# rrwick/Badread

Hardware: AMD Instinct MI355X
Metric: simulated bases/sec (higher is better)
Workload: dtype u32

## Files before the change

### badread_amd/csrc/brx_kernels.h

```cpp
#ifndef BRX_KERNELS_H
#define BRX_KERNELS_H

#include <hip/hip_runtime.h>
#include <stdint.h>

#include "../../include/brx.h"
#include "../../include/brx_spec.h"
#include "brx_align.h"

#define BRX_ALIGN_INTERVAL 25
#define BRX_ALIGN_SIZE 1000
#ifndef BRX_MAX_BASE_SEGS
#define BRX_MAX_BASE_SEGS 64
#endif
#define BRX_OVF_SEGS 4096
#define BRX_OVF_LISTS 64

enum { SEG_REF = 0, SEG_ADAPTER = 1, SEG_RANDOM = 2, SEG_JUNK = 3 };
enum { PC_JUNK = 0, PC_RANDOM = 1, PC_REAL = 2, PC_HAIRPIN = 3 };

struct PSeg { uint32_t w0, start, len, dst; };
struct PPiece { uint32_t w0, left_over; uint64_t start, end; };

struct RS {
// ... 651 lines not shown
                uint8_t kmer[16];
#pragma unroll
                for (int j = 0; j < 16; ++j) kmer[j] = j < k ? F[ipos + j] : 0;
                live = dev_choose_alt(em, kmer, w[2], w[3], rep);
            }
            unsigned long long surv = __ballot(live);
            while (surv) {
                int l = __ffsll((long long)surv) - 1;
                surv &= surv - 1;
                const uint64_t i0 = wave_bcast_u64(ipos, l);
                const double scale = est * brx_sqrt(est);
                for (int j = 0; j < k; ++j) {
                    uint32_t mine = 0;
#pragma unroll
                    for (int jj = 0; jj < 16; ++jj) mine = (jj == j) ? rep[jj] : mine;
                    uint32_t w = wave_bcast_u32(mine, l);
                    if (!w) continue;
                    uint64_t pos = i0 + (uint64_t)j;
                    const uint32_t cur = uni(rp[pos]);
                    if (cur) continue;
                    if (lane == 0) rp[pos] = w;
                    __builtin_amdgcn_fence(__ATOMIC_RELEASE, "workgroup");
                    change += 1;
                    uint32_t len = (w >> 24) & 0x7Fu;
                    errors += (double)(len < 2 ? 1u : len - 1u) * scale;
                    if (change % BRX_ALIGN_INTERVAL == 0) {
                        uint32_t a = 0, b = n;
                        if (n > BRX_ALIGN_SIZE) {
                            uint32_t ww[4];
                            brx_draw4(d.seed, read, BRX_ST_WIN, (uint64_t)nalign, ww);
                            a = (uint32_t)brx_mulhi64(((uint64_t)ww[1] << 32) | ww[0], (uint64_t)n - BRX_ALIGN_SIZE + 1);
                            b = a + BRX_ALIGN_SIZE;
                        }
                        nalign += 1;
                        __builtin_amdgcn_s_waitcnt(0);
                        uint32_t cost = 0;
                        uint32_t tl = wave_join(em, F, rp, a, b, nullptr, &cost);
                        uint32_t ql = b - a;
                        uint64_t qpad = ((uint64_t)ql + 16 + 15) & ~15ull, tpad = ((uint64_t)tl + 16 + 15) & ~15ull;
                        int ncols = 0, nmatch = 0; bool nospace = false;
                        if (qpad + tpad + 64 > win_bytes) nospace = true;
                        else {
                            uint8_t *qb = win, *tbuf = win + qpad;
                            for (uint32_t x = lane; x < ql + 16; x += 64) qb[x] = x < ql ? F[a + x] : 0xFF;
                            for (uint32_t x = lane; x < 16; x += 64) tbuf[tl + x] = 0xFE;
                            wave_join(em, F, rp, a, b, tbuf, nullptr);
                            __builtin_amdgcn_fence(__ATOMIC_RELEASE, "workgroup");
                            __builtin_amdgcn_s_waitcnt(0);
                            uint2 *tb = reinterpret_cast<uint2 *>(win + qpad + tpad);
                            uint64_t cap = (win_bytes - qpad - tpad) / 8;
                            bool ok = brx_wave_align<1>(qb, (int)ql, tbuf, (int)tl, (int)cost, tb, cap, nullptr, &ncols, &nmatch, &nospace,
                                                     nullptr, aclk);
                            if (!ok && !nospace) s.status |= BRX_RS_BAND;
                        }
                        if (nospace) { if (lane == 0) atomicOr(&flags[0], 1u); }
                        double id = ncols ? (double)nmatch / (double)ncols : 0.0;
                        if (n <= BRX_ALIGN_SIZE) errors = (1.0 - id) * dn;
                        else {
                            double est_err = (1.0 - id) * dn;
                            double weight = (double)BRX_ALIGN_SIZE / dn;
                            errors = est_err * weight + errors * (1.0 - weight);
                        }
                    }
                }
                double est2 = 1.0 - errors / dn;
                if ((double)change > 0.9 * dn || est2 <= target) { loops += (uint64_t)l + 2; done = true; break; }
                est = est2;
            }
            if (done) break;
            loops += B;
            if (B < 64) { loops += 1; break; }
        }
        __builtin_amdgcn_s_waitcnt(0);
        uint32_t cost = 0;
        uint32_t m = wave_join(em, F, rp, 0, n, nullptr, &cost);
        uint32_t st = 0, et = 0;
        if (lane < k) { st = rep_len(rp[lane]); et = rep_len(rp[n - k + lane]); }
        st = wave_sum(st); et = wave_sum(et);
        if (lane == 0) {
            RS *o = &rs[r];
            o->status = s.status; o->m = m; o->ub = cost; o->start_trim = st; o->end_trim = et;
            o->loops = (uint32_t)loops; o->changes = change; o->naligns = nalign;
            o->units = 0;
            uint64_t *ck = clk + (uint64_t)r * 8;
            ck[0] = __builtin_amdgcn_s_memtime() - t_begin; ck[1] = aclk[0]; ck[2] = aclk[1];
        }
    }
}

#include "brx_mutate.h"
#include "brx_passes.h"
#include "brx_model.h"
#include "brx_gzip_dev.h"

__global__ void __launch_bounds__(64) k_scan_mut(uint32_t n, RS *rs, const uint32_t *list, uint64_t *totals) {
    const int lane = lane_id();
    uint64_t seq_run = 0, ops_run = 0;
    for (uint32_t base = 0; base < n; base += 64) {
        const uint32_t i = base + lane;
        const uint32_t r = i < n ? list[i] : 0u;
        uint32_t sb = 0, ob = 0;
        if (i < n && rs[r].n) {
            sb = 2u * ((rs[r].m + 16u + 15u) >> 4);
            ob = (rs[r].m + rs[r].n + 16u + 15u) >> 4;
        }
        uint32_t is = wave_incl_scan(sb), io = wave_incl_scan(ob);
        if (i < n) { rs[r].seq_off = (seq_run + is - sb) << 4; rs[r].ops_off = (ops_run + io - ob) << 4; }
        seq_run += wave_bcast_u32(is, 63); ops_run += wave_bcast_u32(io, 63);
    }
    if (lane == 0) { totals[0] = seq_run << 4; totals[1] = ops_run << 4; }
}

__device__ inline int64_t qs_lookup(const brx_qscore_model &qm, uint64_t key) {
    uint64_t h = key * 0x9E3779B97F4A7C15ull;
    uint32_t slot = (uint32_t)(h >> 32) & (qm.hash_size - 1);
    for (;;) {
        uint64_t kk = qm.d_hash_key[slot];
        if (kk == key) return (int64_t)qm.d_hash_row[slot];
        if (kk == ~0ull) return -1;
        slot = (slot + 1) & (qm.hash_size - 1);
    }
}

#define BRX_KL_RETRY 0x10000u
#define BRX_KL_FULL 0x20000u
#define BRX_KL_LANES 0x40000u
#define BRX_KL_QUAD 0x80000u
#include "brx_finlanes.h"
#include "brx_quad.h"

__global__ void __launch_bounds__(64) k_fin_join(BrxDev d, RS *rs, const uint32_t *order, uint32_t q_begin, uint32_t q_end, uint32_t *queue,
                                                  uint64_t seq_base, uint64_t ops_base, const uint8_t *Fbuf, const uint32_t *repl,
                                                  const PPiece *pieces, uint8_t *arena, const uint32_t *F2buf, int fin_lanes, int fin_quad) {
    const int lane = lane_id();
    const brx_error_model &em = d.em;
    for (;;) {
        const uint32_t qi = q_begin + wave_pop(queue);
        if (qi >= q_end) break;
        const uint32_t r = order[qi];
        const RS s = rs[r];
        if (s.n == 0) {
            if (lane == 0) { rs[r].seq_off = seq_base; rs[r].ops_off = ops_base; }
            continue;
        }
        uint8_t *seq = arena + seq_base + s.seq_off;
        wave_join(em, Fbuf + s.F_off, repl + s.F_off, 0, s.n, seq, nullptr);
        for (uint32_t x = lane; x < 16; x += 64) seq[s.m + x] = 0xFE;
        if (lane == 0) {
            const BrxGeom g = brx_make_geom((int)s.m, (int)s.n, (int)s.ub);
            bool junk = false, too_wide;
            if (!d.raw_mode) for (uint32_t i = 0; i < s.n_pieces; ++i) junk |= (pieces[s.piece_off + i].w0 & 3u) == PC_JUNK;
            RS *o = &rs[r];
            o->seq_off = seq_base + s.seq_off; o->ops_off = ops_base + s.ops_off;
            const bool acgt = F2buf[(s.F_off >> 4) + ((s.n + 15u) >> 4)] == 0u;
            const bool lanes = fin_lanes && !junk && acgt && brx_finl_blocks(s.m, s.n, s.ub) > 0;
            const bool quad = fin_quad && !lanes && acgt && g.G == 1 && (brx_quad_words(s.m, s.n, s.ub) & fin_quad) != 0;
            o->klass = (g.G ? (uint32_t)g.G : 0xFFFFu) | (junk ? BRX_KL_FULL : 0u) | (lanes ? BRX_KL_LANES : 0u) | (quad ? BRX_KL_QUAD : 0u);
            o->units = brx_final_units(s.m, s.n, s.ub, junk ? 0 : d.tb_hmul, &too_wide);
            if (too_wide) o->status = s.status | BRX_RS_BAND;
        }
    }
}

__global__ void __launch_bounds__(64, 4) k_fin_lanes(BrxDev d, RS *rs, const uint32_t *list, uint32_t n_list, unsigned long long *ctr,
                                                      const uint64_t *slabs, uint32_t *retries, const uint8_t *Fbuf, uint8_t *seqbuf, uint8_t *opsbuf,
                                                      uint8_t *slab_base, uint64_t *clk) {
    const int lane = lane_id();
    const uint32_t n_groups = (n_list + 63u) >> 6;
    const uint64_t first = uni((uint64_t)atomicAdd(ctr, lane == 0 ? ((1ull << 32) | 1ull) : 0ull));
    uint32_t gi = (uint32_t)first;
    if (gi >= n_groups) return;
    const uint32_t ticket = (uint32_t)(first >> 32);
    const uint64_t slab_at = slabs[ticket], tb_cap = slabs[ticket + 1] - slab_at;
    uint2 *tb = reinterpret_cast<uint2 *>(slab_base) + slab_at;
    for (; gi < n_groups; gi = (uint32_t)uni((uint64_t)atomicAdd(ctr, lane == 0 ? 1ull : 0ull))) {
        const uint32_t idx = gi * 64u + (uint32_t)lane;
        bool valid = idx < n_list;
        const uint32_t r = valid ? list[idx] : 0u;
        RS s;
        if (valid) s = rs[r];
        const uint64_t t_begin = __builtin_amdgcn_s_memtime();
        const uint32_t n = valid ? s.n : 0u, m = valid ? s.m : 0u;
        const uint32_t blocks = wave_max_u32(valid ? (uint32_t)brx_finl_blocks(m, n, s.ub) : 0u);
        const bool fits = brx_finl_units(wave_max_u32(n), blocks) <= tb_cap;
        const uint8_t *F = Fbuf + (valid ? s.F_off : 0ull);
        const uint8_t *seq = seqbuf + (valid ? s.seq_off : 0ull);
        uint8_t *ops_end = opsbuf + (valid ? s.ops_off + (uint64_t)n + (uint64_t)m : 0ull);
        uint32_t ncols = 0, nmatch = 0; bool ok = false;
        brx_lanes_final(valid && fits, seq, (int)m, F, (int)n, valid ? (int)s.ub : 0, tb, ops_end, &ncols, &nmatch, &ok);
        if (valid) {
            RS *o = &rs[r];
            if (!ok) {
                o->klass = (s.klass & ~BRX_KL_LANES) | BRX_KL_RETRY;
                atomicAdd(retries, 1u);
                clk[(uint64_t)r * 8 + 2] = 1;
            } else {
                o->status = s.status;
                o->n_cols = ncols; o->n_match = nmatch;
            }
            uint64_t *ck = clk + (uint64_t)r * 8;
            ck[3] = __builtin_amdgcn_s_memtime() - t_begin; ck[7] = (uint64_t)(s.klass & 0xFFFFu) | 0x20000u;
        }
        __builtin_amdgcn_fence(__ATOMIC_RELEASE, "workgroup");
        __builtin_amdgcn_s_waitcnt(0);
    }
}

template <int G>
__global__ void __launch_bounds__(64, 4) k_fin_quad(BrxDev d, RS *rs, const uint32_t *list, uint32_t n_list, unsigned long long *ctr,
                                                     const uint64_t *slabs, uint32_t *retries, const uint8_t *Fbuf, uint8_t *seqbuf,
                                                     uint8_t *opsbuf, uint8_t *slab_base, uint64_t *clk) {
    const int lane = lane_id();
    const int row = lane >> 4;
    const uint32_t n_groups = (n_list + 3u) >> 2;
    const uint64_t first = uni((uint64_t)atomicAdd(ctr, lane == 0 ? ((1ull << 32) | 1ull) : 0ull));
    uint32_t gi = (uint32_t)first;
    if (gi >= n_groups) return;
    const uint32_t ticket = (uint32_t)(first >> 32);
    const uint64_t slab_at = slabs[ticket], tb_cap = slabs[ticket + 1] - slab_at;
    uint2 *tb = reinterpret_cast<uint2 *>(slab_base) + slab_at;
    for (; gi < n_groups; gi = (uint32_t)uni((uint64_t)atomicAdd(ctr, lane == 0 ? 1ull : 0ull))) {
        const uint32_t idx = gi * 4u + (uint32_t)row;
        const bool valid = idx < n_list;
        const uint32_t r = valid ? list[idx] : 0u;
        RS s;
        if (valid) s = rs[r];
        const uint64_t t_begin = __builtin_amdgcn_s_memtime();
        const uint32_t n = valid ? s.n : 0u, m = valid ? s.m : 0u;
        const uint8_t *F = Fbuf + (valid ? s.F_off : 0ull);
        const uint8_t *seq = seqbuf + (valid ? s.seq_off : 0ull);
        uint8_t *ops_end = opsbuf + (valid ? s.ops_off + (uint64_t)n + (uint64_t)m : 0ull);
        int ncols = 0, nmatch = 0, st = 1;
        brx_quad_align<G>(valid && m > 0 && n > 0, seq, (int)m, F, (int)n, valid ? (int)s.ub : 0,
                          (valid && !(s.klass & BRX_KL_FULL)) ? d.tb_hmul : 0, tb, tb_cap, ops_end, &ncols, &nmatch, &st);
        if (valid && (lane & 15) == 0) {
            RS *o = &rs[r];
            if (st != 0) {
                o->klass = (s.klass & ~BRX_KL_QUAD) | BRX_KL_RETRY;
                atomicAdd(retries, 1u);
                clk[(uint64_t)r * 8 + 2] = 1;
            } else {
                o->status = s.status;
                o->n_cols = (uint32_t)ncols; o->n_match = (uint32_t)nmatch;
            }
            uint64_t *ck = clk + (uint64_t)r * 8;
            ck[3] = __builtin_amdgcn_s_memtime() - t_begin; ck[7] = (uint64_t)(s.klass & 0xFFFFu) | 0x10000u;
        }
        __builtin_amdgcn_fence(__ATOMIC_RELEASE, "workgroup");
        __builtin_amdgcn_s_waitcnt(0);
    }
}

#ifndef BRX_FIN4_WAVES
#define BRX_FIN4_WAVES 4
#endif
template <int MAXG, int GLO, int GHI>
#ifndef BRX_FIN1_WAVES
#define BRX_FIN1_WAVES 5
#endif
#ifndef BRX_FIN2_WAVES
#define BRX_FIN2_WAVES 4
#endif
__global__ void __launch_bounds__(64, (MAXG == 1 ? BRX_FIN1_WAVES : MAXG == 2 ? BRX_FIN2_WAVES : MAXG == 4 ? BRX_FIN4_WAVES : 1)) k_fin_align(BrxDev d, RS *rs, const uint32_t *list, uint32_t n_list,
                                                   unsigned long long *ctr, const uint64_t *slabs, uint32_t *retries, int phase, const uint8_t *Fbuf,
                                                   uint8_t *seqbuf, uint8_t *opsbuf, uint8_t *slab_base, uint64_t *clk) {
    const int lane = lane_id();
    const uint64_t first = uni((uint64_t)atomicAdd(ctr, lane == 0 ? ((1ull << 32) | 1ull) : 0ull));
    uint32_t qi = (uint32_t)first;
    if (qi >= n_list) return;
    const uint32_t ticket = (uint32_t)(first >> 32);
    const uint64_t slab_at = slabs[ticket], tb_cap = slabs[ticket + 1] - slab_at;
    uint2 *tb = reinterpret_cast<uint2 *>(slab_base) + slab_at;
    for (; qi < n_list; qi = (uint32_t)uni((uint64_t)atomicAdd(ctr, lane == 0 ? 1ull : 0ull))) {
        const uint32_t r = list[qi];
        const RS s = rs[r];
        const int klass = (int)(s.klass & 0xFFFFu);
        const uint64_t t_begin = __builtin_amdgcn_s_memtime();
        uint64_t aclk[2] = {0, 0};
        const uint32_t n = s.n, m = s.m;
        const uint8_t *F = Fbuf + s.F_off;
        uint8_t *seq = seqbuf + s.seq_off;
        uint8_t *ops_end = opsbuf + s.ops_off + (uint64_t)n + (uint64_t)m;
        int ncols = 0, nmatch = 0; bool nospace = false;
        const bool ok = brx_wave_align<MAXG, (GLO < MAXG ? GLO : MAXG)>(seq, (int)m, F, (int)n, (int)s.ub, tb, tb_cap, ops_end, &ncols, &nmatch,
                                             &nospace, nullptr, aclk, (phase == 0 && !(s.klass & BRX_KL_FULL)) ? d.tb_hmul : 0);
        if (lane == 0) {
            RS *o = &rs[r];
            if (!ok && phase == 0) {
                o->klass = s.klass | BRX_KL_RETRY;
                atomicAdd(retries, 1u);
                clk[(uint64_t)r * 8 + 2] = 1;
            } else {
                o->status = s.status | (ok ? 0u : BRX_RS_BAND);
                o->n_cols = (uint32_t)ncols; o->n_match = (uint32_t)nmatch;
            }
            uint64_t *ck = clk + (uint64_t)r * 8;
            ck[3] = __builtin_amdgcn_s_memtime() - t_begin; ck[4] = aclk[0]; ck[5] = aclk[1];
            ck[7] = (uint64_t)klass;
        }
    }
}

#define BRX_QS_HOT_MAX 128
#define BRX_QS_PEND 128
__global__ void __launch_bounds__(64) k_fin_qscore(BrxDev d, RS *rs, const uint32_t *order, uint32_t q_begin, uint32_t q_end,
                                                    uint32_t *queue, int phase, int klo, int khi, uint8_t *seqbuf, const uint8_t *opsbuf,
                                                    uint64_t *clk) {
    __shared__ uint32_t qhist[256];
    __shared__ uint32_t hot_thr[BRX_QS_HOT_MAX], hot_score[BRX_QS_HOT_MAX];
    __shared__ uint8_t hot_idx[256];
    __shared__ uint32_t pend_sp[BRX_QS_PEND], pend_h[BRX_QS_PEND], pend_c[BRX_QS_PEND];
    __shared__ uint32_t draw_lds[512];
    const int lane = lane_id();
    const brx_qscore_model &qm = d.qm;
    uint32_t hot_n = 0;
    {
        const int64_t row = qs_lookup(qm, (uint64_t)qm.k << 56);
        if (row >= 0) {
            const uint32_t e0 = qm.d_row_off[row], e1 = qm.d_row_off[row + 1];
            if (e1 - e0 <= BRX_QS_HOT_MAX) {
                hot_n = e1 - e0;
                for (uint32_t x = lane; x < hot_n; x += 64) { hot_thr[x] = qm.d_thr[e0 + x]; hot_score[x] = qm.d_score[e0 + x]; }
            }
        }
        __syncthreads();
        for (uint32_t b = lane; b < 256u && hot_n; b += 64) {
            const uint32_t u = b << 24;
            uint32_t e = 0, hi_ = hot_n - 1;
            while (e < hi_) { const uint32_t mid = (e + hi_) >> 1; if (u < hot_thr[mid]) hi_ = mid; else e = mid + 1; }
            hot_idx[b] = (uint8_t)e;
        }
        __syncthreads();
    }
    for (;;) {
        const uint32_t qi = q_begin + wave_pop(queue);
        if (qi >= q_end) break;
        const uint32_t r = order[qi];
        RS s = rs[r];
        if (s.n == 0) continue;
        if (((s.klass & BRX_KL_RETRY) != 0u) != (phase != 0)) continue;
        if ((int)(s.klass & 0xFFFFu) < klo || (int)(s.klass & 0xFFFFu) > khi) continue;
        const uint64_t t_begin = __builtin_amdgcn_s_memtime();
        const uint64_t read = d.first_read + r;
        const uint32_t n = s.n, m = s.m;
        uint8_t *seq = seqbuf + s.seq_off;
        uint8_t *qual = seq + (((uint64_t)m + 16 + 15) & ~15ull);
        const uint8_t *ops_end = opsbuf + s.ops_off + (uint64_t)n + (uint64_t)m;
        const bool ok = !(s.status & BRX_RS_BAND);
        const uint32_t ncols = s.n_cols;
        const uint8_t *ops = ops_end - ncols;

        for (int b = lane; b < 256; b += 64) qhist[b] = 0;
        __builtin_amdgcn_fence(__ATOMIC_RELEASE, "workgroup");
        __builtin_amdgcn_s_waitcnt(0);
        __syncthreads();

        const uint32_t margin = (uint32_t)(qm.k - 1) / 2;
        const uint32_t maxrun = (1u << qm.gap_bits) - 1u;
        bool qmiss = false;
        uint32_t q_head = 0, q_tail = 0;
        auto slow_lane = [&](uint32_t sp, uint32_t h, uint32_t c) {
            uint64_t opsbits = 0, gapbits = 0;
            {
                uint32_t c0 = c;
                for (uint32_t left = 0; left < h; ) { c0 -= 1u; if (ops[c0] != BRX_OP_D) left += 1u; }
                uint32_t idx = 0, rn = 0;
                for (uint32_t cc = c0; idx < 2u * h + 1u; ++cc) {
                    const uint32_t op = ops[cc];
                    if (op == BRX_OP_D) { rn += 1; continue; }
                    if (idx > 0) { const uint32_t code = rn >= maxrun ? maxrun : rn; gapbits |= (uint64_t)code << (4 * (idx - 1)); }
                    opsbits |= (uint64_t)op << (2 * idx);
                    rn = 0; idx += 1;
                }
            }
            uint32_t score = 0; bool found = false;
            uint32_t hh = h;
            for (;;) {
                uint32_t first = h - hh, cnt = 2 * hh + 1;
                uint64_t key = (uint64_t)cnt << 56;
                int shift = 0;
                for (uint32_t x = 0; x < cnt; ++x) {
                    if (x > 0) { key |= ((gapbits >> (4 * (first + x - 1))) & 15ull) << shift; shift += qm.gap_bits; }
                    key |= ((opsbits >> (2 * (first + x))) & 3ull) << shift; shift += 2;
                }
                int64_t row = qs_lookup(qm, key);
                if (row >= 0) {
                    uint32_t e0 = qm.d_row_off[row], e1 = qm.d_row_off[row + 1];
                    uint32_t w4[4];
                    brx_draw4(d.seed, read, BRX_ST_QS, (uint64_t)(sp >> 2), w4);
                    uint32_t u = w4[sp & 3];
                    uint32_t e = e0, hi_ = e1 - 1;
                    while (e < hi_) { const uint32_t mid = (e + hi_) >> 1; if (u < qm.d_thr[mid]) hi_ = mid; else e = mid + 1; }
                    score = qm.d_score[e]; found = true;
                    break;
                }
                if (hh == 0) break;
                hh -= 1;
            }
            if (!found) qmiss = true;
            qual[sp] = (uint8_t)(score + 33);
            atomicAdd(&qhist[score & 255u], 1u);
        };
        auto drain = [&](uint32_t count) {
            __builtin_amdgcn_fence(__ATOMIC_RELEASE, "workgroup");
            __builtin_amdgcn_s_waitcnt(0);
            __syncthreads();
            if ((uint32_t)lane < count) {
                const uint32_t e = (q_head + (uint32_t)lane) & (BRX_QS_PEND - 1u);
                slow_lane(pend_sp[e], pend_h[e], pend_c[e]);
            }
            q_head += count;
            __syncthreads();
        };
        uint32_t chunks_drawn = 0;
        if (ok) {
            const uint32_t nsteps = (ncols + 63u) >> 6;
            auto load_step = [&](uint32_t step) -> uint32_t {
                const uint32_t c = 64u * step + (uint32_t)lane;
                return (step < nsteps && c < ncols) ? (uint32_t)ops[c] : 0xFFu;
            };
            uint32_t op_cur = load_step(0), op_next = load_step(1);
            unsigned long long e_prev = 0ull, e_cur = __ballot(op_cur == 0u), e_next = 0ull;
            uint32_t sp_base = 0;
            for (uint32_t step = 0; step < nsteps; ++step) {
                const uint32_t op_nn = load_step(step + 2u);
                e_next = __ballot(op_next == 0u);
                const unsigned long long base_m = __ballot(op_cur != BRX_OP_D && op_cur != 0xFFu);
                unsigned long long hot_m = e_cur;
                for (uint32_t dd = 1; dd <= margin; ++dd)
                    hot_m &= ((e_cur >> dd) | (e_next << (64u - dd))) & ((e_cur << dd) | (e_prev >> (64u - dd)));
                while (chunks_drawn <= ((sp_base + 63u) >> 8)) {
                    uint32_t w4[4];
                    brx_draw4(d.seed, read, BRX_ST_QS, (uint64_t)(chunks_drawn * 64u) + (uint64_t)lane, w4);
                    uint32_t *slot = draw_lds + (chunks_drawn & 1u) * 256u + 4u * (uint32_t)lane;
                    slot[0] = w4[0]; slot[1] = w4[1]; slot[2] = w4[2]; slot[3] = w4[3];
                    chunks_drawn += 1u;
                    __builtin_amdgcn_fence(__ATOMIC_RELEASE, "workgroup");
                    __builtin_amdgcn_s_waitcnt(0);
                    __syncthreads();
                }
                const bool valid = ((base_m >> lane) & 1ull) != 0ull;
                const uint32_t sp = sp_base + (uint32_t)__popcll(base_m & ((1ull << lane) - 1ull));
                uint32_t h = margin;
                bool hot = false;
                if (valid) {
                    if (sp < h) h = sp;
                    if (m - 1 - sp < h) h = m - 1 - sp;
                    hot = hot_n && h == margin && ((hot_m >> lane) & 1ull) != 0ull;
                }
                if (hot) {
                    const uint32_t u = draw_lds[((sp >> 8) & 1u) * 256u + (sp & 255u)];
                    uint32_t e = hot_idx[u >> 24];
                    while (e < hot_n - 1u && u >= hot_thr[e]) e += 1u;
                    const uint32_t score = hot_score[e];
                    qual[sp] = (uint8_t)(score + 33);
                    atomicAdd(&qhist[score & 255u], 1u);
                }
                const bool slow = valid && !hot;
                const unsigned long long sm = __ballot(slow);
                if (sm) {
                    if (slow) {
                        const uint32_t e = (q_tail + (uint32_t)__popcll(sm & ((1ull << lane) - 1ull))) & (BRX_QS_PEND - 1u);
                        pend_sp[e] = sp; pend_h[e] = h; pend_c[e] = 64u * step + (uint32_t)lane;
                    }
                    q_tail += (uint32_t)__popcll(sm);
                    if (q_tail - q_head >= 64u) drain(64u);
                }
                sp_base += (uint32_t)__popcll(base_m);
                e_prev = e_cur; e_cur = e_next;
                op_cur = op_next; op_next = op_nn;
            }
        }
        if (q_tail != q_head) drain(q_tail - q_head);
        if (__ballot(qmiss)) s.status |= BRX_RS_QMISS;
        __syncthreads();
        if (lane == 0) {
            double qerr = 0.0;
            for (int q = 0; q < 256; ++q) {
                uint32_t c = qhist[q];
                if (c) qerr += (double)c * brx_exp(-(double)q / 10.0 * 2.302585092994046);
            }
            uint32_t lo = s.start_trim, hi = m >= s.end_trim ? m - s.end_trim : 0;
            if (s.end_trim == 0) hi = 0;
            if (hi < lo) hi = lo;
            RS *o = &rs[r];
            o->status = s.status | ((hi - lo) == 0 ? BRX_RS_EMPTY : 0u);
            o->qerr = qerr;
            o->seq_len = hi - lo;
            clk[(uint64_t)r * 8 + 6] = __builtin_amdgcn_s_memtime() - t_begin;
        }
        __syncthreads();
    }
}

struct CountSink { uint32_t n; __device__ void put(uint8_t) { n++; } };
struct ByteSink { uint8_t *p; uint32_t n; __device__ void put(uint8_t c) { p[n++] = c; } };

template <class S> __device__ void put_str(S &s, const char *t) { while (*t) s.put((uint8_t)*t++); }
template <class S> __device__ void put_dec(S &s, uint64_t v) {
    char buf[24]; int n = 0;
    do { buf[n++] = (char)('0' + (v % 10)); v /= 10; } while (v);
    while (n) s.put((uint8_t)buf[--n]);
}
template <class S> __device__ void put_hex(S &s, uint32_t v, int digits) {
    for (int i = digits - 1; i >= 0; --i) { uint32_t x = (v >> (4 * i)) & 15u; s.put((uint8_t)(x < 10 ? '0' + x : 'a' + x - 10)); }
}
__device__ inline uint64_t milli_round(double v) {
    uint64_t u = brx_d2u(v);
    int e = (int)((u >> 52) & 0x7FF);
    uint64_t mant = u & 0xFFFFFFFFFFFFFull;
    if (e == 0) return 0;
    mant |= 1ull << 52;
    int sh = 1075 - e;
    uint64_t scaled = mant * 1000ull;
    if (sh <= 0) return scaled << (-sh);
    if (sh >= 64) return 0;
    uint64_t q = scaled >> sh, rem = scaled & ((1ull << sh) - 1ull), half = 1ull << (sh - 1);
    if (rem > half || (rem == half && (q & 1ull))) q += 1;
    return q;
}
template <class S>
__device__ void put_uuid(S &s, const BrxDev &d, uint64_t read) {
    uint32_t w[4];
    brx_draw4(d.seed, read, BRX_ST_NAME, 0, w);
    put_hex(s, w[0], 8); s.put('-'); put_hex(s, w[1] >> 16, 4); s.put('-'); put_hex(s, w[1] & 0xFFFFu, 4); s.put('-');
    put_hex(s, w[2] >> 16, 4); s.put('-'); put_hex(s, w[2] & 0xFFFFu, 4); put_hex(s, w[3], 8);
}
template <class S>
__device__ void put_comment(S &s, const BrxDev &d, const RS &r, const PPiece *pieces) {
    for (uint32_t i = 0; i < r.n_pieces; ++i) {
        const PPiece pc = pieces[r.piece_off + i];
        uint32_t type = pc.w0 & 3u, strand = (pc.w0 >> 2) & 1u, contig = pc.w0 >> 3;
        if (i > 0) put_str(s, "chimera ");
        if (type == PC_JUNK) put_str(s, "junk_seq ");
        else if (type == PC_RANDOM) put_str(s, "random_seq ");
        else {
            const brx_contig ct = d.ref.d_contigs[contig];
            for (uint32_t x = 0; x < ct.name_len; ++x) s.put(d.ref.d_names[ct.name_off + x]);
            s.put(','); s.put(strand ? '-' : '+'); put_str(s, "strand,");
            put_dec(s, pc.start); s.put('-'); put_dec(s, pc.end);
            if (type == PC_HAIRPIN) { put_str(s, " (hairpin) 0-"); put_dec(s, pc.left_over); }
            s.put(' ');
        }
    }
    put_str(s, "length="); put_dec(s, r.seq_len);
    put_str(s, " error-free_length="); put_dec(s, r.frag_len);
    put_str(s, " read_identity=");
    double ident = r.n_cols ? (double)r.n_match / (double)r.n_cols : 0.0;
    uint64_t mr = milli_round(ident * 100.0);
    put_dec(s, mr / 1000); s.put('.');
    uint32_t fr = (uint32_t)(mr % 1000);
    s.put((uint8_t)('0' + fr / 100)); s.put((uint8_t)('0' + (fr / 10) % 10)); s.put((uint8_t)('0' + fr % 10));
    s.put('%');
}
template <class S>
__device__ void put_header(S &s, const BrxDev &d, uint64_t read, const RS &r, const PPiece *pieces) {
    s.put('@');
    put_uuid(s, d, read); s.put(' ');
    put_comment(s, d, r, pieces);
    s.put('\n');
}

__global__ void __launch_bounds__(64) k_recsize(BrxDev d, RS *rs, const PPiece *pieces) {
    uint32_t r = blockIdx.x * 64 + threadIdx.x;
    if (r >= d.n_reads) return;
    RS s = rs[r];
    uint32_t len = 0, hl = 0;
    if (s.n && s.seq_len && !(s.status & BRX_RS_NOFRAG)) {
        if (d.raw_mode) len = 2 * s.seq_len;
        else {
            CountSink c; c.n = 0;
            put_header(c, d, d.first_read + r, s, pieces);
            hl = c.n; len = hl + 2 * s.seq_len + 4;
        }
    }
    rs[r].rec_len = len; rs[r].hdr_len = hl;
}

__global__ void __launch_bounds__(64) k_scan_rec(uint32_t n_reads, RS *rs, uint64_t *totals) {
    const int lane = lane_id();
    uint64_t run = 0;
    for (uint32_t base = 0; base < n_reads; base += 64) {
        uint32_t r = base + lane;
        uint32_t len = r < n_reads ? rs[r].rec_len : 0u;
        uint32_t inc = wave_incl_scan(len);
        if (r < n_reads) rs[r].rec_off = run + inc - len;
        run += wave_bcast_u32(inc, 63);
    }
    if (lane == 0) totals[5] = run;
}

__global__ void __launch_bounds__(64) k_emit(BrxDev d, const RS *rs, const PPiece *pieces, const uint8_t *seqbuf, uint8_t *out) {
    const uint32_t r = blockIdx.x;
    const int lane = lane_id();
    const RS s = rs[r];
    if (s.rec_len == 0) return;
    uint8_t *o = out + s.rec_off;
    const uint8_t *seq = seqbuf + s.seq_off + s.start_trim;
    const uint8_t *qual = seqbuf + s.seq_off + (((uint64_t)s.m + 16 + 15) & ~15ull) + s.start_trim;
    const uint32_t L = s.seq_len;
    if (d.raw_mode) {
        for (uint32_t x = lane; x < L; x += 64) { o[x] = seq[x]; o[L + x] = qual[x]; }
        return;
    }
    if (lane == 0) { ByteSink b; b.p = o; b.n = 0; put_header(b, d, d.first_read + r, s, pieces); }
    uint8_t *p = o + s.hdr_len;
    for (uint32_t x = lane; x < L; x += 64) { p[x] = d.ref.sym[seq[x] & 15u]; p[L + 3 + x] = qual[x]; }
    if (lane == 0) { p[L] = '\n'; p[L + 1] = '+'; p[L + 2] = '\n'; p[2 * L + 3] = '\n'; }
}

__global__ void __launch_bounds__(64) k_stats(BrxDev d, const RS *rs, brx_read_stats *out) {
    uint32_t r = blockIdx.x * 64 + threadIdx.x;
    if (r >= d.n_reads) return;
    const RS s = rs[r];
    brx_read_stats o;
    o.status = s.status; o.frag_len = s.frag_len; o.seq_len = s.seq_len; o.n_cols = s.n_cols; o.n_match = s.n_match;
    o.padded_len = s.m; o.loop_count = s.loops; o.change_count = s.changes; o.n_alignments = s.naligns;
    o.rec_len = s.rec_len; o.rec_off = s.rec_off; o.target_identity = s.target; o.qerr_sum = s.qerr;
    out[r] = o;
}

__device__ __forceinline__ uint8_t perm_byte(uint8_t b) {
    switch (b) {
    case 'A': return 0; case 'C': return 1; case 'G': return 2; case 'T': return 3; case 'N': return 4;
    case 0: return 'A'; case 1: return 'C'; case 2: return 'G'; case 3: return 'T'; case 4: return 'N';
    default: return b;
    }
}

__global__ void __launch_bounds__(64) k_align_batch(uint32_t n_pairs, uint32_t p_begin, uint32_t p_end, uint32_t *queue,
                                                     const uint8_t *qs, const uint64_t *q_off, const uint8_t *ts, const uint64_t *t_off,
                                                     const int32_t *k_hint, int32_t *dist, uint32_t *ncols_out, uint32_t *nmatch_out,
                                                     uint8_t *ops_out, const uint64_t *ops_off,
                                                     uint8_t *scr, const uint64_t *scr_off, const uint64_t *scr_bytes,
                                                     uint32_t *prog) {
    const int lane = lane_id();
    for (;;) {
        const uint32_t i = p_begin + wave_pop(queue);
        BRX_PROG(prog, 0, i + 1);
        if (i >= p_end) break;
        const uint32_t Q = (uint32_t)(q_off[i + 1] - q_off[i]), T = (uint32_t)(t_off[i + 1] - t_off[i]);
        const uint8_t *q = qs + q_off[i], *t = ts + t_off[i];
        uint8_t *base = scr + scr_off[i];
        const uint64_t bytes = scr_bytes[i];
        uint64_t qpad = ((uint64_t)Q + 16 + 15) & ~15ull, tpad = ((uint64_t)T + 16 + 15) & ~15ull;
        uint8_t *qb = base, *tbuf = base + qpad;
        for (uint32_t x = lane; x < Q + 16; x += 64) qb[x] = x < Q ? perm_byte(q[x]) : 0xFF;
        for (uint32_t x = lane; x < T + 16; x += 64) tbuf[x] = x < T ? perm_byte(t[x]) : 0xFE;
        __builtin_amdgcn_fence(__ATOMIC_RELEASE, "workgroup");
        __builtin_amdgcn_s_waitcnt(0);
        uint2 *tb = reinterpret_cast<uint2 *>(base + qpad + tpad);
        uint64_t cap = bytes > qpad + tpad ? (bytes - qpad - tpad) / 8 : 0;
        uint8_t *ops_end = ops_out ? ops_out + ops_off[i] + Q + T : nullptr;
        int kh = k_hint[i];
        int maxk = (int)(Q > T ? Q : T);
        int kk = kh >= 0 ? kh : (maxk < 64 ? maxk : 64);
        int nc = 0, nm = 0; bool ok = false, nospace = false;
        BRX_PROG(prog, 1, 1);
        for (int round = 0; round < 40; ++round) {
            BRX_PROG(prog, 2, round + 1);
            ok = uni(brx_wave_align<16>(qb, (int)Q, tbuf, (int)T, kk, tb, cap, ops_end, &nc, &nm, &nospace, prog));
            nc = uni(nc); nm = uni(nm); nospace = uni(nospace);
            if (ok || nospace || kh >= 0 || kk >= maxk) break;
            kk = kk * 2 > maxk ? maxk : kk * 2;
        }
        BRX_PROG(prog, 1, 2);
        if (ok && ops_end) {
            uint8_t *dst = ops_out + ops_off[i];
            const uint8_t *src = ops_end - nc;
            if (dst != src) for (uint32_t base2 = 0; base2 < (uint32_t)nc; base2 += 64) {
                uint32_t x = base2 + lane;
                uint8_t v = x < (uint32_t)nc ? src[x] : 0;
                __builtin_amdgcn_s_waitcnt(0);
                if (x < (uint32_t)nc) dst[x] = v;
                __builtin_amdgcn_fence(__ATOMIC_RELEASE, "workgroup");
                __builtin_amdgcn_s_waitcnt(0);
            }
        }
        BRX_PROG(prog, 1, 3);
        if (lane == 0) {
            dist[i] = ok ? (nc - nm) : (nospace ? -2 : -1);
            ncols_out[i] = ok ? (uint32_t)nc : 0u;
            nmatch_out[i] = ok ? (uint32_t)nm : 0u;
        }
    }
}

#endif
```

Measured before the change: 2.881 billion.

## Split qscore slow path into bitplane mid lanes and LDS op-ring lookups

Reworks the quality-score slow path. Lanes whose full-margin window contains no deletions now build their lookup key straight from per-step X/I ballot bitplanes, and they are queued separately from general lanes. General lanes walk ops from an LDS ring of op bitplanes, falling back to global memory only when the window leaves the held range. The change also reuses the pre-drawn random u instead of redrawing per slow lane, shrinks the key when backing off instead of rebuilding it, tightens waitcnt to LDS only, and parallelises the qerr exp terms across lanes. It adds ballot and LDS work on every step, and the new key construction has to match the old encoding exactly.

```diff
diff --git a/badread_amd/csrc/brx_kernels.h b/badread_amd/csrc/brx_kernels.h
--- a/badread_amd/csrc/brx_kernels.h
+++ b/badread_amd/csrc/brx_kernels.h
@@ -977,15 +977,24 @@
 }
 
 #define BRX_QS_HOT_MAX 128
-#define BRX_QS_PEND 128
+#define BRX_QS_PEND 192
+#ifndef BRX_QS_OPRING
+#define BRX_QS_OPRING 32
+#endif
+#ifndef BRX_QS_REACH
+#define BRX_QS_REACH 32
+#endif
+#define BRX_QS_WAIT_LDS 0xC07F
+static_assert(BRX_QS_REACH >= 1 && BRX_QS_REACH <= 32 && BRX_QS_OPRING >= 2 && (BRX_QS_OPRING & (BRX_QS_OPRING - 1)) == 0, "k_fin_qscore: op planes");
 __global__ void __launch_bounds__(64) k_fin_qscore(BrxDev d, RS *rs, const uint32_t *order, uint32_t q_begin, uint32_t q_end,
                                                     uint32_t *queue, int phase, int klo, int khi, uint8_t *seqbuf, const uint8_t *opsbuf,
                                                     uint64_t *clk) {
     __shared__ uint32_t qhist[256];
     __shared__ uint32_t hot_thr[BRX_QS_HOT_MAX], hot_score[BRX_QS_HOT_MAX];
     __shared__ uint8_t hot_idx[256];
-    __shared__ uint32_t pend_sp[BRX_QS_PEND], pend_h[BRX_QS_PEND], pend_c[BRX_QS_PEND];
-    __shared__ uint32_t draw_lds[512];
+    __shared__ uint32_t pend_sp[BRX_QS_PEND], pend_w[BRX_QS_PEND], pend_u[BRX_QS_PEND];
+    __shared__ unsigned long long op_b0[BRX_QS_OPRING], op_b1[BRX_QS_OPRING];
+    __shared__ union { uint32_t draw[512]; double term[256]; } dq;
     const int lane = lane_id();
     const brx_qscore_model &qm = d.qm;
     uint32_t hot_n = 0;
@@ -1027,64 +1036,104 @@
 
         for (int b = lane; b < 256; b += 64) qhist[b] = 0;
         __builtin_amdgcn_fence(__ATOMIC_RELEASE, "workgroup");
-        __builtin_amdgcn_s_waitcnt(0);
+        __builtin_amdgcn_s_waitcnt(BRX_QS_WAIT_LDS);
         __syncthreads();
 
         const uint32_t margin = (uint32_t)(qm.k - 1) / 2;
         const uint32_t maxrun = (1u << qm.gap_bits) - 1u;
         bool qmiss = false;
-        uint32_t q_head = 0, q_tail = 0;
-        auto slow_lane = [&](uint32_t sp, uint32_t h, uint32_t c) {
-            uint64_t opsbits = 0, gapbits = 0;
-            {
-                uint32_t c0 = c;
-                for (uint32_t left = 0; left < h; ) { c0 -= 1u; if (ops[c0] != BRX_OP_D) left += 1u; }
-                uint32_t idx = 0, rn = 0;
-                for (uint32_t cc = c0; idx < 2u * h + 1u; ++cc) {
-                    const uint32_t op = ops[cc];
-                    if (op == BRX_OP_D) { rn += 1; continue; }
-                    if (idx > 0) { const uint32_t code = rn >= maxrun ? maxrun : rn; gapbits |= (uint64_t)code << (4 * (idx - 1)); }
-                    opsbits |= (uint64_t)op << (2 * idx);
-                    rn = 0; idx += 1;
-                }
-            }
+        uint32_t n_mid = 0, n_gen = 0;
+        uint32_t planes = 0;
+        const uint32_t stride = 2u + (uint32_t)qm.gap_bits;
+        auto lookup_lane = [&](uint64_t key, uint32_t cnt, uint32_t sp, uint32_t u) {
             uint32_t score = 0; bool found = false;
-            uint32_t hh = h;
             for (;;) {
-                uint32_t first = h - hh, cnt = 2 * hh + 1;
-                uint64_t key = (uint64_t)cnt << 56;
-                int shift = 0;
-                for (uint32_t x = 0; x < cnt; ++x) {
-                    if (x > 0) { key |= ((gapbits >> (4 * (first + x - 1))) & 15ull) << shift; shift += qm.gap_bits; }
-                    key |= ((opsbits >> (2 * (first + x))) & 3ull) << shift; shift += 2;
-                }
-                int64_t row = qs_lookup(qm, key);
+                const int64_t row = qs_lookup(qm, key);
                 if (row >= 0) {
-                    uint32_t e0 = qm.d_row_off[row], e1 = qm.d_row_off[row + 1];
-                    uint32_t w4[4];
-                    brx_draw4(d.seed, read, BRX_ST_QS, (uint64_t)(sp >> 2), w4);
-                    uint32_t u = w4[sp & 3];
+                    const uint32_t e0 = qm.d_row_off[row], e1 = qm.d_row_off[row + 1];
                     uint32_t e = e0, hi_ = e1 - 1;
-                    while (e < hi_) { const uint32_t mid = (e + hi_) >> 1; if (u < qm.d_thr[mid]) hi_ = mid; else e = mid + 1; }
-                    score = qm.d_score[e]; found = true;
+                    score = qm.d_score[hi_];
+                    while (e < hi_) {
+                        const uint32_t mid = (e + hi_) >> 1;
+                        const uint32_t t = qm.d_thr[mid], sc = qm.d_score[mid];
+                        if (u < t) { hi_ = mid; score = sc; } else e = mid + 1;
+                    }
+                    found = true;
                     break;
                 }
-                if (hh == 0) break;
-                hh -= 1;
+                if (cnt == 1u) break;
+                cnt -= 2u;
+                key = ((key >> stride) & ((1ull << (cnt * stride - (uint32_t)qm.gap_bits)) - 1ull)) | ((uint64_t)cnt << 56);
             }
             if (!found) qmiss = true;
             qual[sp] = (uint8_t)(score + 33);
             atomicAdd(&qhist[score & 255u], 1u);
         };
-        auto drain = [&](uint32_t count) {
+        auto mid_lane = [&](uint32_t sp, uint32_t w, uint32_t u) {
+            const uint32_t cnt = 2u * margin + 1u;
+            uint64_t key = (uint64_t)cnt << 56;
+            for (uint32_t x = 0; x < cnt; ++x) {
+                const uint32_t op = ((w >> x) & 1u) * BRX_OP_X | ((w >> (16u + x)) & 1u) * BRX_OP_I;
+                key |= (uint64_t)op << (x * stride);
+            }
+            lookup_lane(key, cnt, sp, u);
+        };
+        auto slow_lane = [&](uint32_t sp, uint32_t c, uint32_t u) {
+            uint32_t h = margin;
+            if (sp < h) h = sp;
+            if (m - 1 - sp < h) h = m - 1 - sp;
+            const uint32_t cnt = 2u * h + 1u;
+            auto walk = [&](auto op_at, uint32_t lo, uint32_t hi, uint64_t &key) -> bool {
+                if (c < lo || c >= hi) return false;
+                key = (uint64_t)cnt << 56;
+                uint32_t c0 = c;
+                for (uint32_t left = 0; left < h; ) {
+                    if (c0 <= lo) return false;
+                    c0 -= 1u;
+                    if (op_at(c0) != BRX_OP_D) left += 1u;
+                }
+                uint32_t idx = 0, rn = 0;
+                for (uint32_t cc = c0; idx < cnt; ++cc) {
+                    if (cc >= hi) return false;
+                    const uint32_t op = op_at(cc);
+                    if (op == BRX_OP_D) { rn += 1; continue; }
+                    if (idx > 0) key |= (uint64_t)(rn >= maxrun ? maxrun : rn) << (idx * stride - (uint32_t)qm.gap_bits);
+                    key |= (uint64_t)op << (idx * stride);
+                    rn = 0; idx += 1;
+                }
+                return true;
+            };
+            const uint32_t from = (c > BRX_QS_REACH ? c : BRX_QS_REACH) - BRX_QS_REACH, w = from >> 6, sh = from & 63u;
+            const unsigned long long a0 = op_b0[w & (BRX_QS_OPRING - 1u)], a1 = op_b0[(w + 1u) & (BRX_QS_OPRING - 1u)];
+            const unsigned long long b0 = op_b1[w & (BRX_QS_OPRING - 1u)], b1 = op_b1[(w + 1u) & (BRX_QS_OPRING - 1u)];
+            const unsigned long long l0 = sh ? (a0 >> sh) | (a1 << (64u - sh)) : a0, l1 = sh ? (b0 >> sh) | (b1 << (64u - sh)) : b0;
+            const uint32_t held_lo = 64u * (planes > BRX_QS_OPRING ? planes - BRX_QS_OPRING : 0u), held_hi = 64u * planes;
+            uint64_t key;
+            if (!walk([&](uint32_t cc) { const uint32_t p = cc - from; return (uint32_t)((l0 >> p) & 1ull) | ((uint32_t)((l1 >> p) & 1ull) << 1); },
+                      from > held_lo ? from : held_lo, c + BRX_QS_REACH < held_hi ? c + BRX_QS_REACH : held_hi, key))
+                walk([&](uint32_t cc) { return (uint32_t)ops[cc]; }, 0u, ncols, key);
+            lookup_lane(key, cnt, sp, u);
+        };
+        auto drain_mid = [&](uint32_t count) {
             __builtin_amdgcn_fence(__ATOMIC_RELEASE, "workgroup");
-            __builtin_amdgcn_s_waitcnt(0);
+            __builtin_amdgcn_s_waitcnt(BRX_QS_WAIT_LDS);
             __syncthreads();
+            n_mid -= count;
             if ((uint32_t)lane < count) {
-                const uint32_t e = (q_head + (uint32_t)lane) & (BRX_QS_PEND - 1u);
-                slow_lane(pend_sp[e], pend_h[e], pend_c[e]);
-            }
-            q_head += count;
+                const uint32_t e = n_mid + (uint32_t)lane;
+                mid_lane(pend_sp[e], pend_w[e], pend_u[e]);
+            }
+            __syncthreads();
+        };
+        auto drain_gen = [&](uint32_t count) {
+            __builtin_amdgcn_fence(__ATOMIC_RELEASE, "workgroup");
+            __builtin_amdgcn_s_waitcnt(BRX_QS_WAIT_LDS);
+            __syncthreads();
+            n_gen -= count;
+            if ((uint32_t)lane < count) {
+                const uint32_t e = BRX_QS_PEND - 1u - (n_gen + (uint32_t)lane);
+                slow_lane(pend_sp[e], pend_w[e], pend_u[e]);
+            }
             __syncthreads();
         };
         uint32_t chunks_drawn = 0;
@@ -1096,35 +1145,54 @@
             };
             uint32_t op_cur = load_step(0), op_next = load_step(1);
             unsigned long long e_prev = 0ull, e_cur = __ballot(op_cur == 0u), e_next = 0ull;
+            unsigned long long x_prev = 0ull, x_cur = __ballot(op_cur == BRX_OP_X), x_next = 0ull;
+            unsigned long long i_prev = 0ull, i_cur = __ballot(op_cur == BRX_OP_I), i_next = 0ull;
+            unsigned long long d_prev = 0ull, d_cur = __ballot(op_cur == BRX_OP_D), d_next = 0ull;
+            const uint32_t cut_at = 64u + (uint32_t)lane - margin;
+            auto cut = [&](unsigned long long prev, unsigned long long cur, unsigned long long next) -> uint32_t {
+                const unsigned long long lo = cut_at >= 64u ? cur : prev, hi = cut_at >= 64u ? next : cur;
+                const uint32_t off = cut_at & 63u;
+                const uint32_t v = (uint32_t)(lo >> off) | (off ? (uint32_t)(hi << (64u - off)) : 0u);
+                return v & ((2u << (2u * margin)) - 1u);
+            };
+            if (lane == 0) { op_b0[0] = x_cur | d_cur; op_b1[0] = i_cur | d_cur; }
+            planes = 1u;
             uint32_t sp_base = 0;
             for (uint32_t step = 0; step < nsteps; ++step) {
                 const uint32_t op_nn = load_step(step + 2u);
                 e_next = __ballot(op_next == 0u);
+                x_next = __ballot(op_next == BRX_OP_X);
+                i_next = __ballot(op_next == BRX_OP_I);
+                d_next = __ballot(op_next == BRX_OP_D);
+                if (lane == 0) { op_b0[planes & (BRX_QS_OPRING - 1u)] = x_next | d_next; op_b1[planes & (BRX_QS_OPRING - 1u)] = i_next | d_next; }
+                planes += 1u;
                 const unsigned long long base_m = __ballot(op_cur != BRX_OP_D && op_cur != 0xFFu);
-                unsigned long long hot_m = e_cur;
-                for (uint32_t dd = 1; dd <= margin; ++dd)
+                unsigned long long hot_m = e_cur, dwin_m = d_cur;
+                for (uint32_t dd = 1; dd <= margin; ++dd) {
                     hot_m &= ((e_cur >> dd) | (e_next << (64u - dd))) & ((e_cur << dd) | (e_prev >> (64u - dd)));
+                    dwin_m |= ((d_cur >> dd) | (d_next << (64u - dd))) | ((d_cur << dd) | (d_prev >> (64u - dd)));
+                }
                 while (chunks_drawn <= ((sp_base + 63u) >> 8)) {
                     uint32_t w4[4];
                     brx_draw4(d.seed, read, BRX_ST_QS, (uint64_t)(chunks_drawn * 64u) + (uint64_t)lane, w4);
-                    uint32_t *slot = draw_lds + (chunks_drawn & 1u) * 256u + 4u * (uint32_t)lane;
+                    uint32_t *slot = dq.draw + (chunks_drawn & 1u) * 256u + 4u * (uint32_t)lane;
                     slot[0] = w4[0]; slot[1] = w4[1]; slot[2] = w4[2]; slot[3] = w4[3];
                     chunks_drawn += 1u;
                     __builtin_amdgcn_fence(__ATOMIC_RELEASE, "workgroup");
-                    __builtin_amdgcn_s_waitcnt(0);
+                    __builtin_amdgcn_s_waitcnt(BRX_QS_WAIT_LDS);
                     __syncthreads();
                 }
                 const bool valid = ((base_m >> lane) & 1ull) != 0ull;
-                const uint32_t sp = sp_base + (uint32_t)__popcll(base_m & ((1ull << lane) - 1ull));
-                uint32_t h = margin;
-                bool hot = false;
+                const unsigned long long below = (1ull << lane) - 1ull;
+                const uint32_t sp = sp_base + (uint32_t)__popcll(base_m & below);
+                bool full = false, hot = false;
+                uint32_t u = 0;
                 if (valid) {
-                    if (sp < h) h = sp;
-                    if (m - 1 - sp < h) h = m - 1 - sp;
-                    hot = hot_n && h == margin && ((hot_m >> lane) & 1ull) != 0ull;
+                    full = sp >= margin && m - 1 - sp >= margin;
+                    hot = hot_n && full && ((hot_m >> lane) & 1ull) != 0ull;
+                    u = dq.draw[((sp >> 8) & 1u) * 256u + (sp & 255u)];
                 }
                 if (hot) {
-                    const uint32_t u = draw_lds[((sp >> 8) & 1u) * 256u + (sp & 255u)];
                     uint32_t e = hot_idx[u >> 24];
                     while (e < hot_n - 1u && u >= hot_thr[e]) e += 1u;
                     const uint32_t score = hot_score[e];
@@ -1132,29 +1200,43 @@
                     atomicAdd(&qhist[score & 255u], 1u);
                 }
                 const bool slow = valid && !hot;
-                const unsigned long long sm = __ballot(slow);
-                if (sm) {
-                    if (slow) {
-                        const uint32_t e = (q_tail + (uint32_t)__popcll(sm & ((1ull << lane) - 1ull))) & (BRX_QS_PEND - 1u);
-                        pend_sp[e] = sp; pend_h[e] = h; pend_c[e] = 64u * step + (uint32_t)lane;
+                if (__ballot(slow)) {
+                    const bool mid = slow && full && ((dwin_m >> lane) & 1ull) == 0ull;
+                    const unsigned long long mm = __ballot(mid), gm = __ballot(slow && !mid);
+                    if (mid) {
+                        const uint32_t e = n_mid + (uint32_t)__popcll(mm & below);
+                        pend_sp[e] = sp; pend_u[e] = u;
+                        pend_w[e] = cut(x_prev, x_cur, x_next) | (cut(i_prev, i_cur, i_next) << 16);
+                    } else if (slow) {
+                        const uint32_t e = BRX_QS_PEND - 1u - (n_gen + (uint32_t)__popcll(gm & below));
+                        pend_sp[e] = sp; pend_u[e] = u; pend_w[e] = 64u * step + (uint32_t)lane;
                     }
-                    q_tail += (uint32_t)__popcll(sm);
-                    if (q_tail - q_head >= 64u) drain(64u);
+                    n_mid += (uint32_t)__popcll(mm); n_gen += (uint32_t)__popcll(gm);
+                    if (n_mid >= 64u) drain_mid(64u);
+                    if (n_gen >= 64u) drain_gen(64u);
                 }
                 sp_base += (uint32_t)__popcll(base_m);
                 e_prev = e_cur; e_cur = e_next;
+                x_prev = x_cur; x_cur = x_next;
+                i_prev = i_cur; i_cur = i_next;
+                d_prev = d_cur; d_cur = d_next;
                 op_cur = op_next; op_next = op_nn;
             }
         }
-        if (q_tail != q_head) drain(q_tail - q_head);
+        if (n_mid) drain_mid(n_mid);
+        if (n_gen) drain_gen(n_gen);
         if (__ballot(qmiss)) s.status |= BRX_RS_QMISS;
+        __syncthreads();
+        for (int q = lane; q < 256; q += 64) {
+            const uint32_t c = qhist[q];
+            dq.term[q] = c ? (double)c * brx_exp(-(double)q / 10.0 * 2.302585092994046) : 0.0;
+        }
+        __builtin_amdgcn_fence(__ATOMIC_RELEASE, "workgroup");
+        __builtin_amdgcn_s_waitcnt(BRX_QS_WAIT_LDS);
         __syncthreads();
         if (lane == 0) {
             double qerr = 0.0;
-            for (int q = 0; q < 256; ++q) {
-                uint32_t c = qhist[q];
-                if (c) qerr += (double)c * brx_exp(-(double)q / 10.0 * 2.302585092994046);
-            }
+            for (int q = 0; q < 256; ++q) qerr += dq.term[q];
             uint32_t lo = s.start_trim, hi = m >= s.end_trim ? m - s.end_trim : 0;
             if (s.end_trim == 0) hi = 0;
             if (hi < lo) hi = lo;
```

Result: slower. 2.754 billion (-4.4%).
